# jmoraispk/DeepMIMO

Measured on AMD Instinct MI355X. Metric: user-channels/sec, higher is better.
Workload: dtype f16x3-split MFMA, f32 accumulate

## Files before the change

### deepmimo_amd/csrc/k2_channel_fd_mfma.hip

```cpp
#include "k2_mfma_frag.h"
#include "dmx_tuning.h"
#include <stdlib.h>

namespace dmx {

struct MfmaArgs {
    int64_t user_begin;
    int m_rx, m_tx, ue_mh, bs_mh;
    int M;
    int K;
    const int32_t* sc;
    double inv_n;
    int nblk;
    int rows;
    int n_beams;
    const float2* ftab;
    const int32_t* fexp;
    const float2* gtab;
    const uint2* gpack;
    int adaptive;
    int alias_table;
};

template <bool NT, int NS, bool LW>
__device__ __forceinline__ void mfma_tile(int pt, const unsigned char* Ahi, const unsigned char* Alo, int col, int hh,
                                          const h8 (&Bhi)[4], const h8 (&Blo)[4], const BLane& bl,
                                          __amdgpu_buffer_rsrc_t orsrc, unsigned row_bytes, float oscale) {
    const size_t abase = (size_t)((pt << 5) + col) * ROW_BYTES + (size_t)hh * 16;
    h8 ah[NS], al[NS];
#pragma unroll
    for (int s = 0; s < NS; ++s) {
        ah[s] = *reinterpret_cast<const h8*>(Ahi + abase + s * 32);
        al[s] = *reinterpret_cast<const h8*>(Alo + abase + s * 32);
    }
    __builtin_amdgcn_sched_barrier(0);
    f16v acc;
#pragma unroll
    for (int i = 0; i < 16; ++i) acc[i] = 0.f;
#pragma unroll
    for (int s = 0; s < NS; ++s) {
        acc = __builtin_amdgcn_mfma_f32_32x32x16_f16(ah[s], Bhi[s], acc, 0, 0, 0);
        if (LW && s == NS - 1) continue;
        acc = __builtin_amdgcn_mfma_f32_32x32x16_f16(ah[s], Blo[s], acc, 0, 0, 0);
        acc = __builtin_amdgcn_mfma_f32_32x32x16_f16(al[s], Bhi[s], acc, 0, 0, 0);
    }
    DMX_MFMA_RESULT_GUARD(acc);
    if (bl.kok) {
        const unsigned tile_off = (unsigned)(pt << 5) * row_bytes;
#pragma unroll
        for (int i = 0; i < 16; ++i) {
            const unsigned soff = tile_off + (unsigned)((i & 3) + 8 * (i >> 2)) * row_bytes;
            __builtin_amdgcn_raw_buffer_store_b32(__builtin_bit_cast(unsigned, acc[i] * oscale), orsrc, bl.lane_off, soff, NT ? 2 : 0);
        }
    }
}

template <bool NT>
__device__ __forceinline__ void mfma_tile_rt(int pt, const unsigned char* Ahi, const unsigned char* Alo, int col, int hh, int n_act, int n_full,
                                             const h8 (&Bhi)[4], const h8 (&Blo)[4], const BLane& bl,
                                             __amdgpu_buffer_rsrc_t orsrc, unsigned row_bytes, float oscale) {
    f16v acc;
#pragma unroll
    for (int i = 0; i < 16; ++i) acc[i] = 0.f;
    const size_t abase = (size_t)((pt << 5) + col) * ROW_BYTES + (size_t)hh * 16;
#pragma unroll
    for (int s = 0; s < 4; ++s) {
        if (8 * s < n_act) {
            const h8 ah = *reinterpret_cast<const h8*>(Ahi + abase + s * 32);
            const h8 al = *reinterpret_cast<const h8*>(Alo + abase + s * 32);
            acc = __builtin_amdgcn_mfma_f32_32x32x16_f16(ah, Bhi[s], acc, 0, 0, 0);
            if (s < n_full) {
                acc = __builtin_amdgcn_mfma_f32_32x32x16_f16(ah, Blo[s], acc, 0, 0, 0);
                acc = __builtin_amdgcn_mfma_f32_32x32x16_f16(al, Bhi[s], acc, 0, 0, 0);
            }
        }
    }
    DMX_MFMA_RESULT_GUARD(acc);
    if (bl.kok) {
        const unsigned tile_off = (unsigned)(pt << 5) * row_bytes;
#pragma unroll
        for (int i = 0; i < 16; ++i) {
            const unsigned soff = tile_off + (unsigned)((i & 3) + 8 * (i >> 2)) * row_bytes;
            __builtin_amdgcn_raw_buffer_store_b32(__builtin_bit_cast(unsigned, acc[i] * oscale), orsrc, bl.lane_off, soff, NT ? 2 : 0);
        }
    }
}

template <bool NT, int I0, int I1>
__device__ __forceinline__ void store_rows(const f16v& acc, float oscale, const BLane& bl, __amdgpu_buffer_rsrc_t orsrc,
                                           unsigned tile_off, unsigned row_bytes) {
    if (!bl.kok) return;
#pragma unroll
    for (int i = I0; i < I1; ++i) {
        const unsigned soff = tile_off + (unsigned)((i & 3) + 8 * (i >> 2)) * row_bytes;
        __builtin_amdgcn_raw_buffer_store_b32(__builtin_bit_cast(unsigned, acc[i] * oscale), orsrc, bl.lane_off, soff, NT ? 2 : 0);
    }
}

template <bool NT, int NS, bool STORE_PREV, bool LW>
__device__ __forceinline__ f16v chain_tile(int pt, f16v& prev, const unsigned char* Ahi, const unsigned char* Alo, int col, int hh,
                                           const h8 (&Bhi)[4], const h8 (&Blo)[4], const BLane& bl,
                                           __amdgpu_buffer_rsrc_t orsrc, unsigned row_bytes, float oscale) {
    const size_t abase = (size_t)((pt << 5) + col) * ROW_BYTES + (size_t)hh * 16;
    const unsigned prev_off = (unsigned)((pt - 1) << 5) * row_bytes;
    f16v acc;
#pragma unroll
    for (int i = 0; i < 16; ++i) acc[i] = 0.f;
    h8 ah = *reinterpret_cast<const h8*>(Ahi + abase);
    h8 al = *reinterpret_cast<const h8*>(Alo + abase);
#pragma unroll
    for (int s = 0; s < NS; ++s) {
        acc = __builtin_amdgcn_mfma_f32_32x32x16_f16(ah, Bhi[s], acc, 0, 0, 0);
        if (!(LW && s == NS - 1)) {
            acc = __builtin_amdgcn_mfma_f32_32x32x16_f16(ah, Blo[s], acc, 0, 0, 0);
            acc = __builtin_amdgcn_mfma_f32_32x32x16_f16(al, Bhi[s], acc, 0, 0, 0);
        }
        if (s + 1 < NS) {
            ah = *reinterpret_cast<const h8*>(Ahi + abase + (s + 1) * 32);
            al = *reinterpret_cast<const h8*>(Alo + abase + (s + 1) * 32);
        }
        if constexpr (STORE_PREV) {
            if constexpr (NS == 4) {
                if (s == 0) store_rows<NT, 0, 4>(prev, oscale, bl, orsrc, prev_off, row_bytes);
                if (s == 1) store_rows<NT, 4, 8>(prev, oscale, bl, orsrc, prev_off, row_bytes);
                if (s == 2) store_rows<NT, 8, 12>(prev, oscale, bl, orsrc, prev_off, row_bytes);
                if (s == 3) store_rows<NT, 12, 16>(prev, oscale, bl, orsrc, prev_off, row_bytes);
            } else if constexpr (NS == 3) {
                if (s == 0) store_rows<NT, 0, 6>(prev, oscale, bl, orsrc, prev_off, row_bytes);
                if (s == 1) store_rows<NT, 6, 11>(prev, oscale, bl, orsrc, prev_off, row_bytes);
                if (s == 2) store_rows<NT, 11, 16>(prev, oscale, bl, orsrc, prev_off, row_bytes);
            } else if constexpr (NS == 2) {
                if (s == 0) store_rows<NT, 0, 8>(prev, oscale, bl, orsrc, prev_off, row_bytes);
                if (s == 1) store_rows<NT, 8, 16>(prev, oscale, bl, orsrc, prev_off, row_bytes);
            } else {
                store_rows<NT, 0, 16>(prev, oscale, bl, orsrc, prev_off, row_bytes);
            }
            __builtin_amdgcn_sched_barrier(0);
        }
    }
    DMX_MFMA_RESULT_GUARD(acc);
    return acc;
}

template <bool NT, int NS, bool PIPE, bool LW>
__device__ __forceinline__ void strip_tiles(int ntiles, const unsigned char* Ahi, const unsigned char* Alo, int col, int hh,
                                            const h8 (&Bhi)[4], const h8 (&Blo)[4], const BLane& bl,
                                            __amdgpu_buffer_rsrc_t orsrc, unsigned row_bytes, float oscale) {
    if constexpr (!PIPE) {
        for (int pt = 0; pt < ntiles; ++pt)
            mfma_tile<NT, NS, LW>(pt, Ahi, Alo, col, hh, Bhi, Blo, bl, orsrc, row_bytes, oscale);
        return;
    }
    f16v a0 = {};
    a0 = chain_tile<NT, NS, false, LW>(0, a0, Ahi, Alo, col, hh, Bhi, Blo, bl, orsrc, row_bytes, oscale);
    int pt = 1;
    for (; pt + 1 < ntiles; pt += 2) {
        f16v a1 = chain_tile<NT, NS, true, LW>(pt, a0, Ahi, Alo, col, hh, Bhi, Blo, bl, orsrc, row_bytes, oscale);
        a0 = chain_tile<NT, NS, true, LW>(pt + 1, a1, Ahi, Alo, col, hh, Bhi, Blo, bl, orsrc, row_bytes, oscale);
    }
    if (pt < ntiles) {
        f16v a1 = chain_tile<NT, NS, true, LW>(pt, a0, Ahi, Alo, col, hh, Bhi, Blo, bl, orsrc, row_bytes, oscale);
        store_rows<NT, 0, 16>(a1, oscale, bl, orsrc, (unsigned)(pt << 5) * row_bytes, row_bytes);
    } else {
        store_rows<NT, 0, 16>(a0, oscale, bl, orsrc, (unsigned)((ntiles - 1) << 5) * row_bytes, row_bytes);
    }
}

struct ItemLds {
    unsigned char* Ahi;
    unsigned char* Alo;
    float2* qtab;
    float* crtab;
    float* citab;
    float* misc;
};
__host__ __device__ inline size_t item_lds_bytes(int rows) { return (size_t)2 * rows * ROW_BYTES + LPAD * (8 + 4 + 4) + 16; }
__device__ __forceinline__ ItemLds item_lds(unsigned char* base, int rows) {
    ItemLds L;
    L.Ahi = base;
    L.Alo = base + (size_t)rows * ROW_BYTES;
    L.qtab = reinterpret_cast<float2*>(base + (size_t)2 * rows * ROW_BYTES);
    L.crtab = reinterpret_cast<float*>(L.qtab + LPAD);
    L.citab = L.crtab + LPAD;
    L.misc = L.citab + LPAD;
    return L;
}

struct ItemPos {
    int64_t ul, u;
    int row0, nrows, n_act;
    size_t rb;
};
__device__ __forceinline__ ItemPos item_pos(const WsView& ws, const MfmaArgs& a, int64_t work) {
    ItemPos p;
    p.ul = work / a.nblk;
    const int blk = (int)(work % a.nblk);
    p.u = a.user_begin + p.ul;
    p.row0 = blk * MAX_ROWS;
    p.nrows = (a.M - p.row0) < MAX_ROWS ? (a.M - p.row0) : MAX_ROWS;
    const int n = ws.n_keep[p.u];
    p.n_act = n < LPAD ? n : LPAD;
    p.rb = (size_t)p.u * ws.P;
    return p;
}

template <int NW>
__device__ __forceinline__ void stage_item(const WsView& ws, const MfmaArgs& a, int64_t work, const ItemLds& L) {
    const int tid = threadIdx.x, lane = tid & 63, wave = tid >> 6;
    const ItemPos ip = item_pos(ws, a, work);
    const int n_act = ip.n_act;
    if (n_act == 0) return;
    const float* __restrict__ c_re = ws.c_re + ip.rb;
    const float* __restrict__ c_im = ws.c_im + ip.rb;
    const float* __restrict__ dnp = ws.dn + ip.rb;
    const double* __restrict__ rx_y = ws.rx_y + ip.rb;
    const double* __restrict__ rx_z = ws.rx_z + ip.rb;
    const double* __restrict__ tx_y = ws.tx_y + ip.rb;
    const double* __restrict__ tx_z = ws.tx_z + ip.rb;

    if (wave == 0) {
        float m = 0.f;
        if (lane < n_act) m = fmaxf(fabsf(c_re[lane]), fabsf(c_im[lane]));
        for (int off = 32; off > 0; off >>= 1) m = fmaxf(m, __shfl_xor(m, off));
        const int l0w = ((n_act - 1) >> 3) << 3;
        float a2 = 0.f;
        if (lane < n_act) a2 = fmaf(c_re[lane], c_re[lane], c_im[lane] * c_im[lane]);
        float m2 = a2, mw2 = lane >= l0w ? a2 : 0.f;
        for (int off = 32; off > 0; off >>= 1) { m2 = fmaxf(m2, __shfl_xor(m2, off)); mw2 = fmaxf(mw2, __shfl_xor(mw2, off)); }
        const bool last_weak = a.adaptive && l0w >= 8 && mw2 * 4194304.0f <= m2;
        int e;
        (void)frexpf(m, &e);
        const float gs = ldexpf(1.0f, 10 - e);
        if (lane == 0) L.misc[3] = last_weak ? 1.f : 0.f;
        if (lane < LPAD) {
            const bool ok = lane < n_act;
            const double q = ok ? (double)dnp[lane] * a.inv_n : 0.0;
            const double qh = rint(q * 4096.0) * (1.0 / 4096.0);
            L.qtab[lane] = make_float2((float)qh, (float)(q - qh));
            L.crtab[lane] = ok ? c_re[lane] * gs : 0.f;
            L.citab[lane] = ok ? c_im[lane] * gs : 0.f;
        }
        const int ea = a.n_beams ? 6 - a.fexp[ip.ul] : 6;
        if (a.gtab || a.gpack) e += 2;
        if (lane == 0) { L.misc[0] = ldexpf(1.0f, e - 10 - ea); L.misc[1] = ldexpf(1.0f, ea); L.misc[2] = ldexpf(1.0f, 10 - e); }
    }

    constexpr int LSPLIT = NW / 4, LPER = LPAD / LSPLIT;
    const int r = tid & 255, l0 = (tid >> 8) * LPER;
    if (r >= a.rows) return;
    const int p = ip.row0 + r;
    const bool pok = p < a.M;
    const int ncolA = a.n_beams ? a.n_beams : a.m_tx;
    const int rx = pok ? p / ncolA : 0, tx = pok ? p - rx * ncolA : 0;
    const double yr = (double)(rx % a.ue_mh), zr = (double)(rx / a.ue_mh);
    const double yt = (double)(tx % a.bs_mh), zt = (double)(tx / a.bs_mh);
    h2* rhi = reinterpret_cast<h2*>(L.Ahi + (size_t)r * ROW_BYTES);
    h2* rlo = reinterpret_cast<h2*>(L.Alo + (size_t)r * ROW_BYTES);
    if (a.n_beams) {
        const float2* frow = a.ftab + ((size_t)ip.ul * a.n_beams + tx) * ws.P;
        const float ascale = ldexpf(1.0f, 6 - a.fexp[ip.ul]);
        for (int l = l0; l < l0 + LPER; ++l) {
            h2 vh = {(_Float16)0.f, (_Float16)0.f}, vl = vh;
            if (pok && l < n_act) {
                float s, c;
                sincos_rev(frac_rev(yr * rx_y[l] + zr * rx_z[l]), s, c);
                const float2 f = frow[l];
                split2_f16((c * f.x - s * f.y) * ascale, (c * f.y + s * f.x) * ascale, vh, vl, ws.neg_one);
            }
            rhi[l] = vh;
            rlo[l] = vl;
        }
    } else {
        for (int l = l0; l < l0 + LPER; ++l) {
            h2 vh = {(_Float16)0.f, (_Float16)0.f}, vl = vh;
            if (pok && l < n_act) {
                const double ph = yr * rx_y[l] + zr * rx_z[l] + yt * tx_y[l] + zt * tx_z[l];
                float s, c;
                sincos_rev(frac_rev(ph), s, c);
                split2_f16(c * A_SCALE, s * A_SCALE, vh, vl, ws.neg_one);
            }
            rhi[l] = vh;
            rlo[l] = vl;
        }
    }
}

static constexpr int DMA_SLOT_BYTES = 4096;

__device__ __forceinline__ void dma_strip(const uint2* __restrict__ prow, int K, int kidx0, int nrows, unsigned char* slot, int lane) {
    const int sub = lane >> 3, piece = lane & 7;
#pragma unroll
    for (int j = 0; j < 4; ++j) {
        const int row = 8 * j + sub;
        if (row < nrows) {
            const uint2* g = prow + (size_t)row * K + kidx0 + 2 * piece;
            __builtin_amdgcn_global_load_lds((const __attribute__((address_space(1))) void*)g,
                                             (__attribute__((address_space(3))) void*)(slot + j * 1024), 16, 0, 2);
        }
    }
}

typedef unsigned u4v __attribute__((ext_vector_type(4)));
__device__ __forceinline__ void read_b_slot(const unsigned char* slot, int col, int hh, int c, int n_act, h8 (&Bhi)[4], h8 (&Blo)[4]) {
    const uint32_t a0 = (uint32_t)(size_t)(__attribute__((address_space(3))) const void*)slot + (uint32_t)hh * 512u + (uint32_t)(col >> 1) * 8u;
    const uint32_t a1 = a0 + 2048u;
    const unsigned rot = c ? 16u : 0u, sgn = c ? 0u : 0x80000000u;
#pragma unroll
    for (int half = 0; half < 2; ++half) {
        u4v g[4];
        asm volatile(
            "ds_read2_b64 %0, %4 offset1:16\n\t"
            "ds_read2_b64 %1, %4 offset0:32 offset1:48\n\t"
            "ds_read2_b64 %2, %4 offset0:128 offset1:144\n\t"
            "ds_read2_b64 %3, %4 offset0:160 offset1:176\n\t"
            "s_waitcnt lgkmcnt(0)"
            : "=&v"(g[0]), "=&v"(g[1]), "=&v"(g[2]), "=&v"(g[3]) : "v"(half ? a1 : a0) : "memory");
#pragma unroll
        for (int s2 = 0; s2 < 2; ++s2) {
            const int s = 2 * half + s2;
            Bhi[s] = h8{0, 0, 0, 0, 0, 0, 0, 0};
            Blo[s] = Bhi[s];
            if (8 * s >= n_act) continue;
#pragma unroll
            for (int jj = 0; jj < 4; ++jj) {
                const bool ok = 8 * s + 4 * hh + jj < n_act;
                const unsigned gx = ok ? g[2 * s2 + (jj >> 1)][2 * (jj & 1)] : 0u, gy = ok ? g[2 * s2 + (jj >> 1)][2 * (jj & 1) + 1] : 0u;
                const unsigned xh = __builtin_amdgcn_alignbit(gx, gx, rot) ^ sgn;
                const unsigned xl = __builtin_amdgcn_alignbit(gy, gy, rot) ^ sgn;
                const h2 ph = __builtin_bit_cast(h2, xh), pl2 = __builtin_bit_cast(h2, xl);
                Bhi[s][2 * jj] = ph[0]; Bhi[s][2 * jj + 1] = ph[1];
                Blo[s][2 * jj] = pl2[0]; Blo[s][2 * jj + 1] = pl2[1];
            }
        }
    }
}

__device__ __forceinline__ void wait_dma_behind_stores(int ntiles) {
    if (ntiles >= 4) asm volatile("s_waitcnt vmcnt(63)" ::: "memory");
    else if (ntiles == 3) asm volatile("s_waitcnt vmcnt(48)" ::: "memory");
    else if (ntiles == 2) asm volatile("s_waitcnt vmcnt(32)" ::: "memory");
    else if (ntiles == 1) asm volatile("s_waitcnt vmcnt(16)" ::: "memory");
    else asm volatile("s_waitcnt vmcnt(0)" ::: "memory");
}

template <bool NT, int NW, int MODE, int GSRC>
__device__ __forceinline__ bool consume_item(const WsView& ws, const MfmaArgs& a, float* __restrict__ out, int64_t work,
                                             int64_t next_work, const ItemLds& L, bool prefetched) {
    constexpr int NTHR = NW * 64;
    const int tid = threadIdx.x, lane = tid & 63, wave = tid >> 6;
    const ItemPos ip = item_pos(ws, a, work);
    const size_t twoK = (size_t)2 * a.K;
    float* __restrict__ o = out + ((size_t)ip.ul * a.M + ip.row0) * twoK;
    const int n_act = ip.n_act;
    if (n_act == 0) {
        const size_t nel = (size_t)ip.nrows * twoK;
        for (size_t i = tid; i < nel; i += NTHR) o[i] = 0.f;
        return false;
    }
    const float oscale = L.misc[0];
    const float gscale = L.misc[2];
    const bool last_weak = L.misc[3] != 0.f;
    const float2* grow = GSRC == 1 ? a.gtab + (size_t)ip.ul * ws.P * a.K : nullptr;
    const int64_t tul = a.alias_table ? 0 : ip.ul;
    const uint2* prow = GSRC == 2 ? a.gpack + (size_t)tul * ws.P * a.K : nullptr;
    (void)prefetched;

    const int col = lane & 31, hh = lane >> 5;
    const unsigned row_bytes = (unsigned)twoK * 4u;
    const __amdgpu_buffer_rsrc_t orsrc = __builtin_amdgcn_make_buffer_rsrc(o, 0, (int)((unsigned)ip.nrows * row_bytes), 0x00020000);
    const int nstrips = (int)((twoK + 31) >> 5);
    const int ntiles = (ip.nrows + 31) >> 5;
    unsigned touched = 0;
    bool next_prefetched = false;
    unsigned char* slot = nullptr;
    int nn_next = 0;
    if constexpr (GSRC == 3) {
        __shared__ __attribute__((aligned(16))) unsigned char dma_slots[NW * DMA_SLOT_BYTES];
        slot = dma_slots + wave * DMA_SLOT_BYTES;
        if (next_work >= 0) {
            const int nn = __builtin_amdgcn_readfirstlane(ws.n_keep[a.user_begin + next_work / a.nblk]);
            nn_next = nn < LPAD ? nn : LPAD;
        }
        if (wave < nstrips) {
            if (!prefetched) dma_strip(a.gpack + (size_t)tul * ws.P * a.K, a.K, wave * 16, n_act, slot, lane);
            asm volatile("s_waitcnt vmcnt(0)" ::: "memory");
        }
    }
    for (int strip = wave; strip < nstrips; strip += NW) {
        const BLane bl = b_lane(strip, col, hh, twoK, a.sc);
        h8 Bhi[4], Blo[4];
        if constexpr (GSRC == 3) {
            const uint2* urow = a.gpack + (size_t)tul * ws.P * a.K;
            if (strip != wave) wait_dma_behind_stores(ntiles);
            read_b_slot(slot, col, hh, bl.c, n_act, Bhi, Blo);
            const int ns = strip + NW;
            if (ns < nstrips) {
                dma_strip(urow, a.K, ns * 16, n_act, slot, lane);
            } else if (next_work >= 0) {
                const int64_t nul = a.alias_table ? 0 : next_work / a.nblk;
                dma_strip(a.gpack + (size_t)nul * ws.P * a.K, a.K, wave * 16, nn_next, slot, lane);
                next_prefetched = true;
            }
        } else {
#pragma unroll
            for (int st = 0; st < 4; ++st) {
                if constexpr (GSRC == 2) load_b_step_packed(st, bl, hh, n_act, prow, a.K, Bhi[st], Blo[st]);
                else gen_b_step(ws.neg_one, st, bl, hh, n_act, L.qtab, L.crtab, L.citab, grow, a.K, gscale, Bhi[st], Blo[st]);
            }
        }
        if constexpr (GSRC == 2) {
            asm volatile("" :: "v"(touched), "v"(__builtin_bit_cast(unsigned, h2{Bhi[0][0], Bhi[0][1]})));
            const int ns = strip + NW;
            const uint2* nrow = nullptr;
            const int kmax = a.K - 1;
            if (ns < nstrips) nrow = prow + (size_t)col * a.K + (size_t)(ns * 16 < kmax ? ns * 16 : kmax);
            else if (next_work >= 0) nrow = a.gpack + (size_t)(next_work / a.nblk) * ws.P * a.K + (size_t)col * a.K + (size_t)(wave * 16 < kmax ? wave * 16 : kmax);
            touched = 0;
            if (nrow && hh == 0 && col < ws.P) touched = *reinterpret_cast<const volatile unsigned*>(nrow);
        }
        if constexpr (MODE != 0) {
            constexpr bool PIPE = MODE == 2;
            switch (((n_act + 7) >> 3) + (last_weak ? 4 : 0)) {
                case 1: strip_tiles<NT, 1, PIPE, false>(ntiles, L.Ahi, L.Alo, col, hh, Bhi, Blo, bl, orsrc, row_bytes, oscale); break;
                case 2: strip_tiles<NT, 2, PIPE, false>(ntiles, L.Ahi, L.Alo, col, hh, Bhi, Blo, bl, orsrc, row_bytes, oscale); break;
                case 3: strip_tiles<NT, 3, PIPE, false>(ntiles, L.Ahi, L.Alo, col, hh, Bhi, Blo, bl, orsrc, row_bytes, oscale); break;
                case 4: strip_tiles<NT, 4, PIPE, false>(ntiles, L.Ahi, L.Alo, col, hh, Bhi, Blo, bl, orsrc, row_bytes, oscale); break;
                case 6: strip_tiles<NT, 2, PIPE, true>(ntiles, L.Ahi, L.Alo, col, hh, Bhi, Blo, bl, orsrc, row_bytes, oscale); break;
                case 7: strip_tiles<NT, 3, PIPE, true>(ntiles, L.Ahi, L.Alo, col, hh, Bhi, Blo, bl, orsrc, row_bytes, oscale); break;
                default: strip_tiles<NT, 4, PIPE, true>(ntiles, L.Ahi, L.Alo, col, hh, Bhi, Blo, bl, orsrc, row_bytes, oscale); break;
            }
        } else {
            const int n_full = ((n_act + 7) >> 3) - (last_weak ? 1 : 0);
            for (int pt = 0; pt < ntiles; ++pt)
                mfma_tile_rt<NT>(pt, L.Ahi, L.Alo, col, hh, n_act, n_full, Bhi, Blo, bl, orsrc, row_bytes, oscale);
        }
    }
    return next_prefetched;
}

template <bool NT, int NW, int MODE, int GSRC>
__global__ __launch_bounds__(NW * 64, 4) void k2_fd_mfma(WsView ws, MfmaArgs a, float* __restrict__ out, int64_t total) {
    extern __shared__ __attribute__((aligned(16))) unsigned char smem[];
    const ItemLds L = item_lds(smem, a.rows);
    bool prefetched = false;
    for (int64_t w = blockIdx.x; w < total; w += gridDim.x) {
        stage_item<NW>(ws, a, w, L);
        __syncthreads();
        prefetched = consume_item<NT, NW, MODE, GSRC>(ws, a, out, w, (w + gridDim.x < total) ? w + gridDim.x : (int64_t)-1, L, prefetched);
        __syncthreads();
    }
}

struct BeamArgs {
    int64_t user_begin;
    int m_tx, bs_mh, n_beams;
    const float2* F;
    float2* ftab;
    int32_t* fexp;
};

__global__ __launch_bounds__(256) void k2b_beam_project(WsView ws, BeamArgs a) {
    extern __shared__ __attribute__((aligned(16))) unsigned char smem[];
    float2* atx = reinterpret_cast<float2*>(smem);
    __shared__ float wmax[4];
    const int tid = threadIdx.x;
    const int64_t ul = blockIdx.x, u = a.user_begin + ul;
    const int P = ws.P;
    int n_act = ws.n_keep[u];
    n_act = n_act < LPAD ? n_act : LPAD;
    const size_t rb = (size_t)u * P;
    for (int i = tid; i < a.m_tx * P; i += 256) {
        const int t = i / P, l = i - t * P;
        float s = 0.f, c = 0.f;
        if (l < n_act) {
            const int y = t % a.bs_mh, z = t / a.bs_mh;
            sincos_rev(frac_rev((double)y * ws.tx_y[rb + l] + (double)z * ws.tx_z[rb + l]), s, c);
        }
        atx[i] = make_float2(c, s);
    }
    __syncthreads();
    float m = 0.f;
    for (int i = tid; i < a.n_beams * P; i += 256) {
        const int b = i / P, l = i - b * P;
        float fr = 0.f, fi = 0.f;
        if (l < n_act) {
            const float2* Frow = a.F + (size_t)b * a.m_tx;
            for (int t = 0; t < a.m_tx; ++t) {
                const float2 w = Frow[t], v = atx[t * P + l];
                fr = fmaf(w.x, v.x, fr); fr = fmaf(-w.y, v.y, fr);
                fi = fmaf(w.x, v.y, fi); fi = fmaf(w.y, v.x, fi);
            }
        }
        a.ftab[((size_t)ul * a.n_beams + b) * P + l] = make_float2(fr, fi);
        m = fmaxf(m, fmaxf(fabsf(fr), fabsf(fi)));
    }
    for (int off = 32; off > 0; off >>= 1) m = fmaxf(m, __shfl_xor(m, off));
    if ((tid & 63) == 0) wmax[tid >> 6] = m;
    __syncthreads();
    if (tid == 0) {
        m = fmaxf(fmaxf(wmax[0], wmax[1]), fmaxf(wmax[2], wmax[3]));
        int e = 0;
        if (m > 0.f) (void)frexpf(m, &e);
        a.fexp[ul] = e;
    }
}

template <int NBT>
__global__ __launch_bounds__(256, 2) void k2b_beam_project_mfma(WsView ws, BeamArgs a, int64_t user_count, int kkpad, int fstride) {
    extern __shared__ __attribute__((aligned(16))) unsigned char smem[];
    unsigned char* Fhi = smem;
    unsigned char* Flo = smem + (size_t)NBT * 32 * fstride;
    __shared__ float wmax_s[4];
    const int tid = threadIdx.x, lane = tid & 63, wave = tid >> 6;
    const int B = a.n_beams, P = ws.P;

    float m = 0.f;
    for (int i = tid; i < B * a.m_tx; i += 256) { const float2 w = a.F[i]; m = fmaxf(m, fmaxf(fabsf(w.x), fabsf(w.y))); }
    for (int off = 32; off > 0; off >>= 1) m = fmaxf(m, __shfl_xor(m, off));
    if (lane == 0) wmax_s[wave] = m;
    __syncthreads();
    m = fmaxf(fmaxf(wmax_s[0], wmax_s[1]), fmaxf(wmax_s[2], wmax_s[3]));
    int eF = 0;
    if (m > 0.f) (void)frexpf(m, &eF);
    const float sF = ldexpf(1.0f, 10 - eF);
    const float oscale = ldexpf(1.0f, eF - 10 - 6);
    const int half_kk = kkpad >> 1;
    for (int i = tid; i < NBT * 32 * half_kk; i += 256) {
        const int b = i / half_kk, t = i - b * half_kk;
        h2 vh = {(_Float16)0.f, (_Float16)0.f}, vl = vh;
        if (b < B && t < a.m_tx) {
            const float2 w = a.F[(size_t)b * a.m_tx + t];
            split2_f16(w.x * sF, w.y * sF, vh, vl, ws.neg_one);
        }
        reinterpret_cast<h2*>(Fhi + (size_t)b * fstride)[t] = vh;
        reinterpret_cast<h2*>(Flo + (size_t)b * fstride)[t] = vl;
    }
    __syncthreads();

    const int colr = lane & 31, hh = lane >> 5, c = lane & 1;
    const int ksteps = kkpad >> 4;
    for (int64_t ul = (int64_t)blockIdx.x * 4 + wave; ul < user_count; ul += (int64_t)gridDim.x * 4) {
        const int64_t u = a.user_begin + ul;
        int n_act = ws.n_keep[u];
        n_act = n_act < LPAD ? n_act : LPAD;
        const size_t rb = (size_t)u * P;
        float* fout = reinterpret_cast<float*>(a.ftab + (size_t)ul * B * P);
        float wmax = 0.f;
        const int nct = (2 * n_act + 31) >> 5;
        for (int ct = 0; ct < nct; ++ct) {
            const int col = (ct << 5) + colr, l = col >> 1;
            const bool lok = l < n_act;
            const double ty = lok ? ws.tx_y[rb + l] : 0.0, tz = lok ? ws.tx_z[rb + l] : 0.0;
            f16v acc[NBT];
#pragma unroll
            for (int bt = 0; bt < NBT; ++bt)
#pragma unroll
                for (int i = 0; i < 16; ++i) acc[bt][i] = 0.f;
            for (int s = 0; s < ksteps; ++s) {
                float mr[2], mi[2], orr[2], oi[2];
#pragma unroll
                for (int t = 0; t < 2; ++t) {
                    const int tx = 8 * s + 4 * hh + 2 * c + t;
                    float sn = 0.f, cs = 0.f;
                    if (lok && tx < a.m_tx) {
                        sincos_rev(frac_rev((double)(tx % a.bs_mh) * ty + (double)(tx / a.bs_mh) * tz), sn, cs);
                        sn *= A_SCALE; cs *= A_SCALE;
                    }
                    mr[t] = cs; mi[t] = sn;
                }
#pragma unroll
                for (int t = 0; t < 2; ++t) { orr[t] = __shfl_xor(mr[t], 1); oi[t] = __shfl_xor(mi[t], 1); }
                float gr[4], gi[4];
                gr[0] = c ? orr[0] : mr[0]; gi[0] = c ? oi[0] : mi[0];
                gr[1] = c ? orr[1] : mr[1]; gi[1] = c ? oi[1] : mi[1];
                gr[2] = c ? mr[0] : orr[0]; gi[2] = c ? mi[0] : oi[0];
                gr[3] = c ? mr[1] : orr[1]; gi[3] = c ? mi[1] : oi[1];
                h8 Bh, Bl;
#pragma unroll
                for (int jj = 0; jj < 4; ++jj) {
                    const float e0 = c ? gi[jj] : gr[jj];
                    const float e1 = c ? gr[jj] : -gi[jj];
                    h2 ph, pl2;
                    split2_f16(e0, e1, ph, pl2, ws.neg_one);
                    Bh[2 * jj] = ph[0]; Bh[2 * jj + 1] = ph[1];
                    Bl[2 * jj] = pl2[0]; Bl[2 * jj + 1] = pl2[1];
                }
#pragma unroll
                for (int bt = 0; bt < NBT; ++bt) {
                    const size_t aoff = (size_t)((bt << 5) + colr) * fstride + (size_t)s * 32 + (size_t)hh * 16;
                    const h8 ah = *reinterpret_cast<const h8*>(Fhi + aoff);
                    const h8 al = *reinterpret_cast<const h8*>(Flo + aoff);
                    acc[bt] = __builtin_amdgcn_mfma_f32_32x32x16_f16(ah, Bh, acc[bt], 0, 0, 0);
                    acc[bt] = __builtin_amdgcn_mfma_f32_32x32x16_f16(ah, Bl, acc[bt], 0, 0, 0);
                    acc[bt] = __builtin_amdgcn_mfma_f32_32x32x16_f16(al, Bh, acc[bt], 0, 0, 0);
                }
            }
            DMX_MFMA_RESULT_GUARD_FENCED();
#pragma unroll
            for (int bt = 0; bt < NBT; ++bt)
// ... 194 lines not shown
```

### deepmimo_amd/csrc/k2_mfma_frag.h

```cpp
#pragma once
#include "dmx_common.h"

namespace dmx {

typedef _Float16 h8 __attribute__((ext_vector_type(8)));
typedef _Float16 h2 __attribute__((ext_vector_type(2)));
typedef float f16v __attribute__((ext_vector_type(16)));

static constexpr int ROW_BYTES = 144;
static constexpr int MAX_ROWS = 256;
static constexpr int MFMA_LDS_MAX = 80 * 1024;
static constexpr int LPAD = 32;
static constexpr float A_SCALE = 64.0f;

#define DMX_MFMA_RESULT_GUARD(acc) asm volatile("s_nop 4" : "+v"(acc))
#define DMX_MFMA_RESULT_GUARD2(acc_a, acc_b) asm volatile("s_nop 4" : "+v"(acc_a), "+v"(acc_b))
#define DMX_MFMA_RESULT_GUARD_FENCED() do { __builtin_amdgcn_sched_barrier(0); asm volatile("s_nop 4"); __builtin_amdgcn_sched_barrier(0); } while (0)

typedef __fp16 hp2 __attribute__((ext_vector_type(2)));
__device__ __forceinline__ void split2_f16(float x0, float x1, h2& hi, h2& lo, float m1) {
    const hp2 h = __builtin_amdgcn_cvt_pkrtz(x0, x1);
    const h2 hh = __builtin_bit_cast(h2, h);
    const float r0 = __builtin_fmaf((float)hh[0], m1, x0);
    const float r1 = __builtin_fmaf((float)hh[1], m1, x1);
    const hp2 l = __builtin_amdgcn_cvt_pkrtz(r0, r1);
    hi = hh;
    lo = __builtin_bit_cast(h2, l);
}

struct BLane {
    int kidx, c;
    bool kok;
    unsigned lane_off;
    float kl, kf;
};

__device__ __forceinline__ BLane b_lane(int strip, int col, int hh, size_t twoK, const int32_t* __restrict__ sc) {
    BLane b;
    const int ncol = (strip << 5) + col;
    b.kidx = ncol >> 1; b.c = ncol & 1;
    b.kok = (size_t)ncol < twoK;
    b.lane_off = ((unsigned)(4 * hh) * (unsigned)twoK + (unsigned)ncol) * 4u;
    const int kki = b.kok ? sc[b.kidx] : 0;
    b.kl = (float)(kki & 4095);
    b.kf = (float)kki;
    return b;
}

__device__ __forceinline__ void gen_b_step(float m1, int s, const BLane& bl, int hh, int n_act, const float2* qtab, const float* crtab,
                                           const float* citab, const float2* __restrict__ grow, int K, float gs,
                                           h8& Bhi, h8& Blo) {
    Bhi = h8{0, 0, 0, 0, 0, 0, 0, 0};
    Blo = Bhi;
    if (8 * s >= n_act) return;
    const int c = bl.c;
    float mr[2], mi[2], orr[2], oi[2];
#pragma unroll
    for (int t = 0; t < 2; ++t) {
        const int pl = 8 * s + 4 * hh + 2 * c + t;
        if (grow) {
            float2 g = make_float2(0.f, 0.f);
            if (bl.kok && pl < n_act) g = grow[(size_t)pl * K + bl.kidx];
            mr[t] = g.x * gs; mi[t] = g.y * gs;
        } else {
            float sn, cs;
            const float2 q = qtab[pl];
            const float p1 = q.x * bl.kl;
            sincos_rev(fmaf(q.y, bl.kf, p1 - rintf(p1)), sn, cs);
            const float cr = crtab[pl], ci = citab[pl];
            mr[t] = cr * cs + ci * sn;
            mi[t] = ci * cs - cr * sn;
        }
    }
#pragma unroll
    for (int t = 0; t < 2; ++t) { orr[t] = __shfl_xor(mr[t], 1); oi[t] = __shfl_xor(mi[t], 1); }
    float gr[4], gi[4];
    gr[0] = c ? orr[0] : mr[0]; gi[0] = c ? oi[0] : mi[0];
    gr[1] = c ? orr[1] : mr[1]; gi[1] = c ? oi[1] : mi[1];
    gr[2] = c ? mr[0] : orr[0]; gi[2] = c ? mi[0] : oi[0];
    gr[3] = c ? mr[1] : orr[1]; gi[3] = c ? mi[1] : oi[1];
#pragma unroll
    for (int jj = 0; jj < 4; ++jj) {
        const float e0 = c ? gi[jj] : gr[jj];
        const float e1 = c ? gr[jj] : -gi[jj];
        h2 ph, pl2;
        split2_f16(e0, e1, ph, pl2, m1);
        Bhi[2 * jj] = ph[0]; Bhi[2 * jj + 1] = ph[1];
        Blo[2 * jj] = pl2[0]; Blo[2 * jj + 1] = pl2[1];
    }
}

__device__ __forceinline__ void load_b_step_packed(int s, const BLane& bl, int hh, int n_act, const uint2* __restrict__ prow, int K,
                                                   h8& Bhi, h8& Blo) {
    Bhi = h8{0, 0, 0, 0, 0, 0, 0, 0};
    Blo = Bhi;
    if (8 * s >= n_act) return;
    const unsigned rot = bl.c ? 16u : 0u, sgn = bl.c ? 0u : 0x80000000u;
    uint2 g[4];
#pragma unroll
    for (int jj = 0; jj < 4; ++jj) {
        const int pl = 8 * s + 4 * hh + jj;
        g[jj] = make_uint2(0u, 0u);
        if (bl.kok && pl < n_act) g[jj] = prow[(size_t)pl * K + bl.kidx];
    }
#pragma unroll
    for (int jj = 0; jj < 4; ++jj) {
        const unsigned xh = __builtin_amdgcn_alignbit(g[jj].x, g[jj].x, rot) ^ sgn;
        const unsigned xl = __builtin_amdgcn_alignbit(g[jj].y, g[jj].y, rot) ^ sgn;
        const h2 ph = __builtin_bit_cast(h2, xh), pl2 = __builtin_bit_cast(h2, xl);
        Bhi[2 * jj] = ph[0]; Bhi[2 * jj + 1] = ph[1];
        Blo[2 * jj] = pl2[0]; Blo[2 * jj + 1] = pl2[1];
    }
}

struct BeamTabs {
    const float2* ftab;
    const int32_t* fexp;
};

}
```

Before: 6.076 million.

## Pack partial K-tail hi/lo split terms into fewer MFMA steps

Adds a tail-packing scheme for the f16x3-split MFMA GEMM. When the number of active paths is not a multiple of 8, the hi/hi, hi/lo and lo/hi products for the remaining 1-5 paths are interleaved into one or two 16-deep K slices. The A rows in LDS are rewritten to match, so the tail costs 1-2 MFMAs instead of 3. The GSRC==0 path now dispatches on a compile-time (nf,nx) form and regenerates B per strip. This adds template instantiations, an LDS rewrite in the staging step and extra code complexity.

Result: faster. 6.236 million (median of 6 runs) (+2.6%).

```diff
diff --git a/deepmimo_amd/csrc/k2_channel_fd_mfma.hip b/deepmimo_amd/csrc/k2_channel_fd_mfma.hip
--- a/deepmimo_amd/csrc/k2_channel_fd_mfma.hip
+++ b/deepmimo_amd/csrc/k2_channel_fd_mfma.hip
@@ -22,28 +22,35 @@
     int alias_table;
 };
 
-template <bool NT, int NS, bool LW>
+static constexpr int mfmas_before(int s, int NF) { return s < NF ? 3 * s : 3 * NF + (s - NF); }
+
+template <bool NT, int NF, int NX>
 __device__ __forceinline__ void mfma_tile(int pt, const unsigned char* Ahi, const unsigned char* Alo, int col, int hh,
                                           const h8 (&Bhi)[4], const h8 (&Blo)[4], const BLane& bl,
                                           __amdgpu_buffer_rsrc_t orsrc, unsigned row_bytes, float oscale) {
+    constexpr int NT1 = NF < 4 ? NF : 3;
     const size_t abase = (size_t)((pt << 5) + col) * ROW_BYTES + (size_t)hh * 16;
-    h8 ah[NS], al[NS];
-#pragma unroll
-    for (int s = 0; s < NS; ++s) {
+    h8 ah[NF + NX], al[NF > 0 ? NF : 1];
+#pragma unroll
+    for (int s = 0; s < NF; ++s) {
         ah[s] = *reinterpret_cast<const h8*>(Ahi + abase + s * 32);
         al[s] = *reinterpret_cast<const h8*>(Alo + abase + s * 32);
     }
+#pragma unroll
+    for (int x = 0; x < NX; ++x) ah[NF + x] = *reinterpret_cast<const h8*>((x ? Alo : Ahi) + abase + NT1 * 32);
     __builtin_amdgcn_sched_barrier(0);
     f16v acc;
 #pragma unroll
     for (int i = 0; i < 16; ++i) acc[i] = 0.f;
 #pragma unroll
-    for (int s = 0; s < NS; ++s) {
+    for (int s = 0; s < NF; ++s) {
         acc = __builtin_amdgcn_mfma_f32_32x32x16_f16(ah[s], Bhi[s], acc, 0, 0, 0);
-        if (LW && s == NS - 1) continue;
         acc = __builtin_amdgcn_mfma_f32_32x32x16_f16(ah[s], Blo[s], acc, 0, 0, 0);
         acc = __builtin_amdgcn_mfma_f32_32x32x16_f16(al[s], Bhi[s], acc, 0, 0, 0);
     }
+#pragma unroll
+    for (int x = 0; x < NX; ++x)
+        acc = __builtin_amdgcn_mfma_f32_32x32x16_f16(ah[NF + x], x ? Blo[NT1] : Bhi[NT1], acc, 0, 0, 0);
     DMX_MFMA_RESULT_GUARD(acc);
     if (bl.kok) {
         const unsigned tile_off = (unsigned)(pt << 5) * row_bytes;
@@ -56,7 +63,7 @@
 }
 
 template <bool NT>
-__device__ __forceinline__ void mfma_tile_rt(int pt, const unsigned char* Ahi, const unsigned char* Alo, int col, int hh, int n_act, int n_full,
+__device__ __forceinline__ void mfma_tile_rt(int pt, const unsigned char* Ahi, const unsigned char* Alo, int col, int hh, int nf, int nx,
                                              const h8 (&Bhi)[4], const h8 (&Blo)[4], const BLane& bl,
                                              __amdgpu_buffer_rsrc_t orsrc, unsigned row_bytes, float oscale) {
     f16v acc;
@@ -65,13 +72,13 @@
     const size_t abase = (size_t)((pt << 5) + col) * ROW_BYTES + (size_t)hh * 16;
 #pragma unroll
     for (int s = 0; s < 4; ++s) {
-        if (8 * s < n_act) {
+        if (s < nf + (nx > 0 ? 1 : 0)) {
             const h8 ah = *reinterpret_cast<const h8*>(Ahi + abase + s * 32);
             const h8 al = *reinterpret_cast<const h8*>(Alo + abase + s * 32);
             acc = __builtin_amdgcn_mfma_f32_32x32x16_f16(ah, Bhi[s], acc, 0, 0, 0);
-            if (s < n_full) {
-                acc = __builtin_amdgcn_mfma_f32_32x32x16_f16(ah, Blo[s], acc, 0, 0, 0);
-                acc = __builtin_amdgcn_mfma_f32_32x32x16_f16(al, Bhi[s], acc, 0, 0, 0);
+            if (s < nf || nx > 1) {
+                acc = __builtin_amdgcn_mfma_f32_32x32x16_f16(s < nf ? ah : al, Blo[s], acc, 0, 0, 0);
+                if (s < nf) acc = __builtin_amdgcn_mfma_f32_32x32x16_f16(al, Bhi[s], acc, 0, 0, 0);
             }
         }
     }
@@ -86,21 +93,24 @@
     }
 }
 
-template <bool NT, int I0, int I1>
+template <bool NT>
 __device__ __forceinline__ void store_rows(const f16v& acc, float oscale, const BLane& bl, __amdgpu_buffer_rsrc_t orsrc,
-                                           unsigned tile_off, unsigned row_bytes) {
+                                           unsigned tile_off, unsigned row_bytes, int i0, int i1) {
     if (!bl.kok) return;
 #pragma unroll
-    for (int i = I0; i < I1; ++i) {
+    for (int i = 0; i < 16; ++i) {
+        if (i < i0 || i >= i1) continue;
         const unsigned soff = tile_off + (unsigned)((i & 3) + 8 * (i >> 2)) * row_bytes;
         __builtin_amdgcn_raw_buffer_store_b32(__builtin_bit_cast(unsigned, acc[i] * oscale), orsrc, bl.lane_off, soff, NT ? 2 : 0);
     }
 }
 
-template <bool NT, int NS, bool STORE_PREV, bool LW>
+template <bool NT, int NF, int NX, bool STORE_PREV>
 __device__ __forceinline__ f16v chain_tile(int pt, f16v& prev, const unsigned char* Ahi, const unsigned char* Alo, int col, int hh,
                                            const h8 (&Bhi)[4], const h8 (&Blo)[4], const BLane& bl,
                                            __amdgpu_buffer_rsrc_t orsrc, unsigned row_bytes, float oscale) {
+    constexpr int NR = NF + NX, NM = 3 * NF + NX;
+    constexpr int NT1 = NF < 4 ? NF : 3;
     const size_t abase = (size_t)((pt << 5) + col) * ROW_BYTES + (size_t)hh * 16;
     const unsigned prev_off = (unsigned)((pt - 1) << 5) * row_bytes;
     f16v acc;
@@ -109,32 +119,25 @@
     h8 ah = *reinterpret_cast<const h8*>(Ahi + abase);
     h8 al = *reinterpret_cast<const h8*>(Alo + abase);
 #pragma unroll
-    for (int s = 0; s < NS; ++s) {
-        acc = __builtin_amdgcn_mfma_f32_32x32x16_f16(ah, Bhi[s], acc, 0, 0, 0);
-        if (!(LW && s == NS - 1)) {
+    for (int s = 0; s < NR; ++s) {
+        if (s < NF) {
+            acc = __builtin_amdgcn_mfma_f32_32x32x16_f16(ah, Bhi[s], acc, 0, 0, 0);
             acc = __builtin_amdgcn_mfma_f32_32x32x16_f16(ah, Blo[s], acc, 0, 0, 0);
             acc = __builtin_amdgcn_mfma_f32_32x32x16_f16(al, Bhi[s], acc, 0, 0, 0);
-        }
-        if (s + 1 < NS) {
-            ah = *reinterpret_cast<const h8*>(Ahi + abase + (s + 1) * 32);
-            al = *reinterpret_cast<const h8*>(Alo + abase + (s + 1) * 32);
+        } else {
+            acc = __builtin_amdgcn_mfma_f32_32x32x16_f16(ah, s == NF ? Bhi[NT1] : Blo[NT1], acc, 0, 0, 0);
+        }
+        if (s + 1 < NR) {
+            if (s + 1 < NF) {
+                ah = *reinterpret_cast<const h8*>(Ahi + abase + (s + 1) * 32);
+                al = *reinterpret_cast<const h8*>(Alo + abase + (s + 1) * 32);
+            } else {
+                ah = *reinterpret_cast<const h8*>((s + 1 == NF ? Ahi : Alo) + abase + NT1 * 32);
+            }
         }
         if constexpr (STORE_PREV) {
-            if constexpr (NS == 4) {
-                if (s == 0) store_rows<NT, 0, 4>(prev, oscale, bl, orsrc, prev_off, row_bytes);
-                if (s == 1) store_rows<NT, 4, 8>(prev, oscale, bl, orsrc, prev_off, row_bytes);
-                if (s == 2) store_rows<NT, 8, 12>(prev, oscale, bl, orsrc, prev_off, row_bytes);
-                if (s == 3) store_rows<NT, 12, 16>(prev, oscale, bl, orsrc, prev_off, row_bytes);
-            } else if constexpr (NS == 3) {
-                if (s == 0) store_rows<NT, 0, 6>(prev, oscale, bl, orsrc, prev_off, row_bytes);
-                if (s == 1) store_rows<NT, 6, 11>(prev, oscale, bl, orsrc, prev_off, row_bytes);
-                if (s == 2) store_rows<NT, 11, 16>(prev, oscale, bl, orsrc, prev_off, row_bytes);
-            } else if constexpr (NS == 2) {
-                if (s == 0) store_rows<NT, 0, 8>(prev, oscale, bl, orsrc, prev_off, row_bytes);
-                if (s == 1) store_rows<NT, 8, 16>(prev, oscale, bl, orsrc, prev_off, row_bytes);
-            } else {
-                store_rows<NT, 0, 16>(prev, oscale, bl, orsrc, prev_off, row_bytes);
-            }
+            store_rows<NT>(prev, oscale, bl, orsrc, prev_off, row_bytes, (16 * mfmas_before(s, NF) + NM - 1) / NM,
+                           (16 * mfmas_before(s + 1, NF) + NM - 1) / NM);
             __builtin_amdgcn_sched_barrier(0);
         }
     }
@@ -142,27 +145,27 @@
     return acc;
 }
 
-template <bool NT, int NS, bool PIPE, bool LW>
+template <bool NT, int NF, int NX, bool PIPE>
 __device__ __forceinline__ void strip_tiles(int ntiles, const unsigned char* Ahi, const unsigned char* Alo, int col, int hh,
                                             const h8 (&Bhi)[4], const h8 (&Blo)[4], const BLane& bl,
                                             __amdgpu_buffer_rsrc_t orsrc, unsigned row_bytes, float oscale) {
     if constexpr (!PIPE) {
         for (int pt = 0; pt < ntiles; ++pt)
-            mfma_tile<NT, NS, LW>(pt, Ahi, Alo, col, hh, Bhi, Blo, bl, orsrc, row_bytes, oscale);
+            mfma_tile<NT, NF, NX>(pt, Ahi, Alo, col, hh, Bhi, Blo, bl, orsrc, row_bytes, oscale);
         return;
     }
     f16v a0 = {};
-    a0 = chain_tile<NT, NS, false, LW>(0, a0, Ahi, Alo, col, hh, Bhi, Blo, bl, orsrc, row_bytes, oscale);
+    a0 = chain_tile<NT, NF, NX, false>(0, a0, Ahi, Alo, col, hh, Bhi, Blo, bl, orsrc, row_bytes, oscale);
     int pt = 1;
     for (; pt + 1 < ntiles; pt += 2) {
-        f16v a1 = chain_tile<NT, NS, true, LW>(pt, a0, Ahi, Alo, col, hh, Bhi, Blo, bl, orsrc, row_bytes, oscale);
-        a0 = chain_tile<NT, NS, true, LW>(pt + 1, a1, Ahi, Alo, col, hh, Bhi, Blo, bl, orsrc, row_bytes, oscale);
+        f16v a1 = chain_tile<NT, NF, NX, true>(pt, a0, Ahi, Alo, col, hh, Bhi, Blo, bl, orsrc, row_bytes, oscale);
+        a0 = chain_tile<NT, NF, NX, true>(pt + 1, a1, Ahi, Alo, col, hh, Bhi, Blo, bl, orsrc, row_bytes, oscale);
     }
     if (pt < ntiles) {
-        f16v a1 = chain_tile<NT, NS, true, LW>(pt, a0, Ahi, Alo, col, hh, Bhi, Blo, bl, orsrc, row_bytes, oscale);
-        store_rows<NT, 0, 16>(a1, oscale, bl, orsrc, (unsigned)(pt << 5) * row_bytes, row_bytes);
+        f16v a1 = chain_tile<NT, NF, NX, true>(pt, a0, Ahi, Alo, col, hh, Bhi, Blo, bl, orsrc, row_bytes, oscale);
+        store_rows<NT>(a1, oscale, bl, orsrc, (unsigned)(pt << 5) * row_bytes, row_bytes, 0, 16);
     } else {
-        store_rows<NT, 0, 16>(a0, oscale, bl, orsrc, (unsigned)((ntiles - 1) << 5) * row_bytes, row_bytes);
+        store_rows<NT>(a0, oscale, bl, orsrc, (unsigned)((ntiles - 1) << 5) * row_bytes, row_bytes, 0, 16);
     }
 }
 
@@ -204,10 +207,20 @@
     return p;
 }
 
-template <int NW>
+struct TailForm { int nf, nx; bool packed; };
+__device__ __forceinline__ TailForm tail_form(int n_act, bool weak, bool packable) {
+    const int nfull = n_act >> 3, r = n_act & 7;
+    if (packable && r >= 1 && (r <= 2 || (r <= 5 && !weak))) return {nfull, r <= 2 ? 1 : 2, true};
+    if (weak) return {r ? nfull : nfull - 1, 1, false};
+    return {r ? nfull + 1 : nfull, 0, false};
+}
+__device__ __forceinline__ int tail_form_code(const TailForm& f) { return (f.nf << 3) | (f.packed ? 4 : 0) | f.nx; }
+
+template <int NW, bool PACK>
 __device__ __forceinline__ void stage_item(const WsView& ws, const MfmaArgs& a, int64_t work, const ItemLds& L) {
     const int tid = threadIdx.x, lane = tid & 63, wave = tid >> 6;
     const ItemPos ip = item_pos(ws, a, work);
+    const unsigned ulane = (unsigned)lane;
     const int n_act = ip.n_act;
     if (n_act == 0) return;
     const float* __restrict__ c_re = ws.c_re + ip.rb;
@@ -218,27 +231,32 @@
     const double* __restrict__ tx_y = ws.tx_y + ip.rb;
     const double* __restrict__ tx_z = ws.tx_z + ip.rb;
 
+    bool last_weak = false;
+    if (a.adaptive) {
+        const int l0w = ((n_act - 1) >> 3) << 3;
+        float a2 = 0.f;
+        if (lane < n_act) a2 = fmaf(c_re[ulane], c_re[ulane], c_im[ulane] * c_im[ulane]);
+        float m2 = a2, mw2 = lane >= l0w ? a2 : 0.f;
+        for (int off = 32; off > 0; off >>= 1) { m2 = fmaxf(m2, __shfl_xor(m2, off)); mw2 = fmaxf(mw2, __shfl_xor(mw2, off)); }
+        last_weak = l0w >= 8 && __builtin_amdgcn_readfirstlane(mw2 * 4194304.0f <= m2);
+    }
+    const TailForm tf = tail_form(n_act, last_weak, PACK);
+
     if (wave == 0) {
         float m = 0.f;
-        if (lane < n_act) m = fmaxf(fabsf(c_re[lane]), fabsf(c_im[lane]));
+        if (lane < n_act) m = fmaxf(fabsf(c_re[ulane]), fabsf(c_im[ulane]));
         for (int off = 32; off > 0; off >>= 1) m = fmaxf(m, __shfl_xor(m, off));
-        const int l0w = ((n_act - 1) >> 3) << 3;
-        float a2 = 0.f;
-        if (lane < n_act) a2 = fmaf(c_re[lane], c_re[lane], c_im[lane] * c_im[lane]);
-        float m2 = a2, mw2 = lane >= l0w ? a2 : 0.f;
-        for (int off = 32; off > 0; off >>= 1) { m2 = fmaxf(m2, __shfl_xor(m2, off)); mw2 = fmaxf(mw2, __shfl_xor(mw2, off)); }
-        const bool last_weak = a.adaptive && l0w >= 8 && mw2 * 4194304.0f <= m2;
         int e;
         (void)frexpf(m, &e);
         const float gs = ldexpf(1.0f, 10 - e);
-        if (lane == 0) L.misc[3] = last_weak ? 1.f : 0.f;
+        if (lane == 0) L.misc[3] = (float)tail_form_code(tf);
         if (lane < LPAD) {
             const bool ok = lane < n_act;
-            const double q = ok ? (double)dnp[lane] * a.inv_n : 0.0;
+            const double q = ok ? (double)dnp[ulane] * a.inv_n : 0.0;
             const double qh = rint(q * 4096.0) * (1.0 / 4096.0);
             L.qtab[lane] = make_float2((float)qh, (float)(q - qh));
-            L.crtab[lane] = ok ? c_re[lane] * gs : 0.f;
-            L.citab[lane] = ok ? c_im[lane] * gs : 0.f;
+            L.crtab[lane] = ok ? c_re[ulane] * gs : 0.f;
+            L.citab[lane] = ok ? c_im[ulane] * gs : 0.f;
         }
         const int ea = a.n_beams ? 6 - a.fexp[ip.ul] : 6;
         if (a.gtab || a.gpack) e += 2;
@@ -283,6 +301,28 @@
             rlo[l] = vl;
         }
     }
+    if (tf.packed) {
+        const int lt = n_act & ~7;
+        if (lt >= l0 && lt < l0 + LPER) {
+            typedef unsigned u4 __attribute__((ext_vector_type(4)));
+            typedef __attribute__((address_space(3))) u4 lu4;
+            const unsigned roff = (unsigned)(threadIdx.x & 255) * ROW_BYTES + (unsigned)lt * 4u;
+            lu4* ph = reinterpret_cast<lu4*>((__attribute__((address_space(3))) unsigned char*)L.Ahi + roff);
+            lu4* pl = reinterpret_cast<lu4*>((__attribute__((address_space(3))) unsigned char*)L.Alo + roff);
+            const u4 h0 = ph[0], h1 = ph[1], l0v = pl[0];
+            const unsigned hi[5] = {h0[0], h0[1], h0[2], h0[3], h1[0]};
+            const unsigned lo[5] = {l0v[0], l0v[1], l0v[2], l0v[3], pl[1][0]};
+            unsigned q[16];
+#pragma unroll
+            for (int t = 0; t < 5; ++t) { q[3 * t] = hi[t]; q[3 * t + 1] = hi[t]; q[3 * t + 2] = lo[t]; }
+            q[15] = 0u;
+            const int r3 = 3 * (n_act - lt);
+#pragma unroll
+            for (int i = 0; i < 16; ++i) q[i] = i < r3 ? q[i] : 0u;
+            ph[0] = u4{q[0], q[1], q[2], q[3]};  ph[1] = u4{q[4], q[5], q[6], q[7]};
+            pl[0] = u4{q[8], q[9], q[10], q[11]}; pl[1] = u4{q[12], q[13], q[14], q[15]};
+        }
+    }
 }
 
 static constexpr int DMA_SLOT_BYTES = 4096;
@@ -341,6 +381,39 @@
     else if (ntiles == 2) asm volatile("s_waitcnt vmcnt(32)" ::: "memory");
     else if (ntiles == 1) asm volatile("s_waitcnt vmcnt(16)" ::: "memory");
     else asm volatile("s_waitcnt vmcnt(0)" ::: "memory");
+}
+
+template <bool NT, int NW, int MODE, int NF, int NX>
+__device__ __forceinline__ void strips_form(const WsView& ws, const MfmaArgs& a, const ItemLds& L, int n_act, bool packed,
+                                            const float2* __restrict__ grow, float gscale, int nstrips, int ntiles,
+                                            __amdgpu_buffer_rsrc_t orsrc, unsigned row_bytes, float oscale) {
+    const int lane = threadIdx.x & 63, wave = threadIdx.x >> 6;
+    const int col = lane & 31, hh = lane >> 5;
+    const size_t twoK = (size_t)2 * a.K;
+    for (int strip = wave; strip < nstrips; strip += NW) {
+        const BLane bl = b_lane(strip, col, hh, twoK, a.sc);
+        h8 Bhi[4], Blo[4];
+#pragma unroll
+        for (int st = 0; st < NF; ++st)
+            gen_b_step(ws.neg_one, st, bl, hh, n_act, L.qtab, L.crtab, L.citab, grow, a.K, gscale, Bhi[st], Blo[st]);
+        if constexpr (NX > 0) {
+            constexpr int S = NF < 4 ? NF : 3;
+            if (packed) {
+                Bhi[S] = gen_b_tail_step<0>(ws.neg_one, bl, hh, NF << 3, n_act, L.qtab, L.crtab, L.citab, grow, a.K, gscale);
+                if constexpr (NX > 1)
+                    Blo[S] = gen_b_tail_step<1>(ws.neg_one, bl, hh, NF << 3, n_act, L.qtab, L.crtab, L.citab, grow, a.K, gscale);
+            } else {
+                h8 unused;
+                gen_b_step(ws.neg_one, S, bl, hh, n_act, L.qtab, L.crtab, L.citab, grow, a.K, gscale, Bhi[S], unused);
+            }
+        }
+        if constexpr (MODE != 0) {
+            strip_tiles<NT, NF, NX, MODE == 2>(ntiles, L.Ahi, L.Alo, col, hh, Bhi, Blo, bl, orsrc, row_bytes, oscale);
+        } else {
+            for (int pt = 0; pt < ntiles; ++pt)
+                mfma_tile_rt<NT>(pt, L.Ahi, L.Alo, col, hh, NF, NX, Bhi, Blo, bl, orsrc, row_bytes, oscale);
+        }
+    }
 }
 
 template <bool NT, int NW, int MODE, int GSRC>
@@ -359,7 +432,9 @@
     }
     const float oscale = L.misc[0];
     const float gscale = L.misc[2];
-    const bool last_weak = L.misc[3] != 0.f;
+    const int form = __builtin_amdgcn_readfirstlane((int)L.misc[3]);
+    const int nf = form >> 3, nx = form & 3;
+    const bool packed = (form & 4) != 0;
     const float2* grow = GSRC == 1 ? a.gtab + (size_t)ip.ul * ws.P * a.K : nullptr;
     const int64_t tul = a.alias_table ? 0 : ip.ul;
     const uint2* prow = GSRC == 2 ? a.gpack + (size_t)tul * ws.P * a.K : nullptr;
@@ -370,6 +445,17 @@
     const __amdgpu_buffer_rsrc_t orsrc = __builtin_amdgcn_make_buffer_rsrc(o, 0, (int)((unsigned)ip.nrows * row_bytes), 0x00020000);
     const int nstrips = (int)((twoK + 31) >> 5);
     const int ntiles = (ip.nrows + 31) >> 5;
+    if constexpr (GSRC == 0) {
+#define DMX_FORM(NF, NX) case (NF << 2 | NX): strips_form<NT, NW, MODE, NF, NX>(ws, a, L, n_act, packed, grow, gscale, nstrips, ntiles, orsrc, row_bytes, oscale); break;
+        switch ((nf << 2) | nx) {
+            DMX_FORM(1, 0) DMX_FORM(2, 0) DMX_FORM(3, 0)
+            DMX_FORM(0, 1) DMX_FORM(1, 1) DMX_FORM(2, 1) DMX_FORM(3, 1)
+            DMX_FORM(0, 2) DMX_FORM(1, 2) DMX_FORM(2, 2) DMX_FORM(3, 2)
+            default: strips_form<NT, NW, MODE, 4, 0>(ws, a, L, n_act, packed, grow, gscale, nstrips, ntiles, orsrc, row_bytes, oscale); break;
+        }
+#undef DMX_FORM
+        return false;
+    }
     unsigned touched = 0;
     bool next_prefetched = false;
     unsigned char* slot = nullptr;
@@ -420,19 +506,15 @@
         }
         if constexpr (MODE != 0) {
             constexpr bool PIPE = MODE == 2;
-            switch (((n_act + 7) >> 3) + (last_weak ? 4 : 0)) {
-                case 1: strip_tiles<NT, 1, PIPE, false>(ntiles, L.Ahi, L.Alo, col, hh, Bhi, Blo, bl, orsrc, row_bytes, oscale); break;
-                case 2: strip_tiles<NT, 2, PIPE, false>(ntiles, L.Ahi, L.Alo, col, hh, Bhi, Blo, bl, orsrc, row_bytes, oscale); break;
-                case 3: strip_tiles<NT, 3, PIPE, false>(ntiles, L.Ahi, L.Alo, col, hh, Bhi, Blo, bl, orsrc, row_bytes, oscale); break;
-                case 4: strip_tiles<NT, 4, PIPE, false>(ntiles, L.Ahi, L.Alo, col, hh, Bhi, Blo, bl, orsrc, row_bytes, oscale); break;
-                case 6: strip_tiles<NT, 2, PIPE, true>(ntiles, L.Ahi, L.Alo, col, hh, Bhi, Blo, bl, orsrc, row_bytes, oscale); break;
-                case 7: strip_tiles<NT, 3, PIPE, true>(ntiles, L.Ahi, L.Alo, col, hh, Bhi, Blo, bl, orsrc, row_bytes, oscale); break;
-                default: strip_tiles<NT, 4, PIPE, true>(ntiles, L.Ahi, L.Alo, col, hh, Bhi, Blo, bl, orsrc, row_bytes, oscale); break;
+            switch (nf) {
+                case 1: strip_tiles<NT, 1, 0, PIPE>(ntiles, L.Ahi, L.Alo, col, hh, Bhi, Blo, bl, orsrc, row_bytes, oscale); break;
+                case 2: strip_tiles<NT, 2, 0, PIPE>(ntiles, L.Ahi, L.Alo, col, hh, Bhi, Blo, bl, orsrc, row_bytes, oscale); break;
+                case 3: strip_tiles<NT, 3, 0, PIPE>(ntiles, L.Ahi, L.Alo, col, hh, Bhi, Blo, bl, orsrc, row_bytes, oscale); break;
+                default: strip_tiles<NT, 4, 0, PIPE>(ntiles, L.Ahi, L.Alo, col, hh, Bhi, Blo, bl, orsrc, row_bytes, oscale); break;
             }
         } else {
-            const int n_full = ((n_act + 7) >> 3) - (last_weak ? 1 : 0);
             for (int pt = 0; pt < ntiles; ++pt)
-                mfma_tile_rt<NT>(pt, L.Ahi, L.Alo, col, hh, n_act, n_full, Bhi, Blo, bl, orsrc, row_bytes, oscale);
+                mfma_tile_rt<NT>(pt, L.Ahi, L.Alo, col, hh, nf, 0, Bhi, Blo, bl, orsrc, row_bytes, oscale);
         }
     }
     return next_prefetched;
@@ -444,7 +526,7 @@
     const ItemLds L = item_lds(smem, a.rows);
     bool prefetched = false;
     for (int64_t w = blockIdx.x; w < total; w += gridDim.x) {
-        stage_item<NW>(ws, a, w, L);
+        stage_item<NW, GSRC == 0>(ws, a, w, L);
         __syncthreads();
         prefetched = consume_item<NT, NW, MODE, GSRC>(ws, a, out, w, (w + gridDim.x < total) ? w + gridDim.x : (int64_t)-1, L, prefetched);
         __syncthreads();
diff --git a/deepmimo_amd/csrc/k2_mfma_frag.h b/deepmimo_amd/csrc/k2_mfma_frag.h
--- a/deepmimo_amd/csrc/k2_mfma_frag.h
+++ b/deepmimo_amd/csrc/k2_mfma_frag.h
@@ -47,6 +47,29 @@
     return b;
 }
 
+__device__ __forceinline__ void b_phasor(int pl, const BLane& bl, int n_act, const float2* qtab, const float* crtab,
+                                         const float* citab, const float2* __restrict__ grow, int K, float gs, float& mr, float& mi) {
+    if (grow) {
+        float2 g = make_float2(0.f, 0.f);
+        if (bl.kok && pl < n_act) g = grow[(size_t)pl * K + bl.kidx];
+        mr = g.x * gs; mi = g.y * gs;
+    } else {
+        float sn, cs;
+        const float2 q = qtab[pl];
+        const float p1 = q.x * bl.kl;
+        sincos_rev(fmaf(q.y, bl.kf, p1 - rintf(p1)), sn, cs);
+        const float cr = crtab[pl], ci = citab[pl];
+        mr = cr * cs + ci * sn;
+        mi = ci * cs - cr * sn;
+    }
+}
+
+__device__ __forceinline__ void b_pair(int c, float gr, float gi, h2& hi, h2& lo, float m1) {
+    const float e0 = c ? gi : gr;
+    const float e1 = c ? gr : -gi;
+    split2_f16(e0, e1, hi, lo, m1);
+}
+
 __device__ __forceinline__ void gen_b_step(float m1, int s, const BLane& bl, int hh, int n_act, const float2* qtab, const float* crtab,
                                            const float* citab, const float2* __restrict__ grow, int K, float gs,
                                            h8& Bhi, h8& Blo) {
@@ -56,22 +79,7 @@
     const int c = bl.c;
     float mr[2], mi[2], orr[2], oi[2];
 #pragma unroll
-    for (int t = 0; t < 2; ++t) {
-        const int pl = 8 * s + 4 * hh + 2 * c + t;
-        if (grow) {
-            float2 g = make_float2(0.f, 0.f);
-            if (bl.kok && pl < n_act) g = grow[(size_t)pl * K + bl.kidx];
-            mr[t] = g.x * gs; mi[t] = g.y * gs;
-        } else {
-            float sn, cs;
-            const float2 q = qtab[pl];
-            const float p1 = q.x * bl.kl;
-            sincos_rev(fmaf(q.y, bl.kf, p1 - rintf(p1)), sn, cs);
-            const float cr = crtab[pl], ci = citab[pl];
-            mr[t] = cr * cs + ci * sn;
-            mi[t] = ci * cs - cr * sn;
-        }
-    }
+    for (int t = 0; t < 2; ++t) b_phasor(8 * s + 4 * hh + 2 * c + t, bl, n_act, qtab, crtab, citab, grow, K, gs, mr[t], mi[t]);
 #pragma unroll
     for (int t = 0; t < 2; ++t) { orr[t] = __shfl_xor(mr[t], 1); oi[t] = __shfl_xor(mi[t], 1); }
     float gr[4], gi[4];
@@ -81,13 +89,35 @@
     gr[3] = c ? mr[1] : orr[1]; gi[3] = c ? mi[1] : oi[1];
 #pragma unroll
     for (int jj = 0; jj < 4; ++jj) {
-        const float e0 = c ? gi[jj] : gr[jj];
-        const float e1 = c ? gr[jj] : -gi[jj];
         h2 ph, pl2;
-        split2_f16(e0, e1, ph, pl2, m1);
+        b_pair(c, gr[jj], gi[jj], ph, pl2, m1);
         Bhi[2 * jj] = ph[0]; Bhi[2 * jj + 1] = ph[1];
         Blo[2 * jj] = pl2[0]; Blo[2 * jj + 1] = pl2[1];
     }
+}
+
+template <int M>
+__device__ __forceinline__ h8 gen_b_tail_step(float m1, const BLane& bl, int hh, int lt, int n_act, const float2* qtab, const float* crtab,
+                                              const float* citab, const float2* __restrict__ grow, int K, float gs) {
+    const int c = bl.c;
+    const int t0 = hh ? (8 * M + 4) / 3 : (8 * M) / 3;
+    float mr, mi;
+    b_phasor(lt + t0 + c, bl, n_act, qtab, crtab, citab, grow, K, gs, mr, mi);
+    const float orr = __shfl_xor(mr, 1), oi = __shfl_xor(mi, 1);
+    h2 hi[2], lo[2];
+    b_pair(c, c ? orr : mr, c ? oi : mi, hi[0], lo[0], m1);
+    b_pair(c, c ? mr : orr, c ? mi : oi, hi[1], lo[1], m1);
+    h8 B;
+#pragma unroll
+    for (int j = 0; j < 4; ++j) {
+        const int q0 = 8 * M + j, q1 = 8 * M + 4 + j;
+        const int u0 = q0 / 3 - (8 * M) / 3, u1 = q1 / 3 - (8 * M + 4) / 3;
+        const h2 v0 = q0 % 3 == 1 ? lo[u0] : hi[u0];
+        const h2 v1 = q1 % 3 == 1 ? lo[u1] : hi[u1];
+        const h2 v = hh ? v1 : v0;
+        B[2 * j] = v[0]; B[2 * j + 1] = v[1];
+    }
+    return B;
 }
 
 __device__ __forceinline__ void load_b_step_packed(int s, const BLane& bl, int hh, int n_act, const uint2* __restrict__ prow, int K,
```
